# refresh-bio/fqsqueezer

Hardware: AMD Instinct MI355X
Metric: Mbases/s compressed (DNA stream, SE sorted) (higher is better)
Workload: dtype u64; 1 GPU; 1000000x150bp SE, G=7500000 (seed 2+rank), -om s -gs 8 -qm n -im n; workers_T=64, blocks=256, per_gpu=one independent file per GPU

## Files before the change

fqsqueezer_amd/codec.py:

```python
from __future__ import annotations

import ctypes as C
import os
from typing import List, Optional

import numpy as np

_PKG = os.path.dirname(os.path.abspath(__file__))
DEFAULT_LIB = os.path.join(_PKG, "libfqsx.so")

STAT_NAMES = ["gprobe", "gslot", "lprobe", "lslot", "gins", "gins_slot", "siv_words", "ctx_slots",
              "coded", "lins", "mail", "bases", "siv_saved", "dec_refetch"]


class FqsxError(RuntimeError):
    pass


def _load(path: str):
    if not os.path.exists(path):
        raise FqsxError(f"{path} not found: build it with `python -c 'import __graft_entry__ as g; g.build()'` "
                        "(hipcc --offload-arch=gfx950); there is no CPU fallback")
    try:
        import torch
    except ImportError:
        pass
    lib = C.CDLL(path)
    lib.fqsx_dna_create.restype = C.c_int
    lib.fqsx_dna_create.argtypes = [C.c_char_p, C.c_int, C.POINTER(C.c_void_p)]
    if hasattr(lib, "fqsx_dna_create_on_partition"):
        lib.fqsx_dna_create_on_partition.restype = C.c_int
        lib.fqsx_dna_create_on_partition.argtypes = [C.c_char_p, C.c_int, C.c_uint32, C.c_uint32, C.POINTER(C.c_void_p)]
    lib.fqsx_dna_destroy.argtypes = [C.c_void_p]
    lib.fqsx_dna_encode_block.restype = C.c_int
    lib.fqsx_dna_encode_block.argtypes = [C.c_void_p, C.c_void_p, C.c_void_p, C.c_uint32, C.c_uint32,
# ... 759 lines not shown
```

fqsqueezer_amd/csrc/fqsx_dev.h:

```cpp
#pragma once
#include "fqsx_layout.h"
#include "fqsx_rc.h"

#define FQSX_RR 6u
#define FQSX_SW 4u
#define FQSX_NSC 3u
#define FQSX_SCR FQSX_NSC
#define FQSX_RQ 256u
struct SpecBuf {
  u32 h_read, h_i0, h_n;
  u32 h_epoch;
  u32 h_pub;
  u32 h_fix_lane, h_fix_end;
  u32 h_pq_lo[2];
  u32 h_np, h_nlp;
  u64 h_ns, h_nls;
  u64 sp_sdir[6][FQSX_SPEC];
  u64 sp_src[6][FQSX_SPEC];
  u8 sp_scur[6][FQSX_SPEC];
  u64 sp_key[10][FQSX_SPEC];
  u8 sp_kind[FQSX_SPEC];
  u64 sp_cq[FQSX_SPEC];
  u8 sp_lvz[FQSX_SPEC];
  u8 sp_flag[FQSX_SPEC];
  u8 sp_rsym[FQSX_SPEC];
  u8 sp_rep[FQSX_SPEC];
  u8 sp_nrun[FQSX_SPEC];
  u64 pv_b[FQSX_SPEC], pv_s[FQSX_SPEC], pv_pd[FQSX_SPEC], pv_pr[FQSX_SPEC];
  u8 pv_flag[FQSX_SPEC];
  u32 sx_lb[FQSX_SPEC];
  u64 sx_s[FQSX_SPEC];
  u64 sx_ls[FQSX_SPEC];
  u8 sx_flag[FQSX_SPEC];
  u8 rr_idx[FQSX_SPEC];
  u32 rr_front;
  u64 rr_res[FQSX_RR][64];
  u64 rr_hit[FQSX_RR];
  u64 rr_ns[FQSX_RR];
  u64 rc_hit[FQSX_SPEC];
  u64 rc_val[FQSX_SPEC][3];
  u32 rc_ns[FQSX_SPEC];
  u8 ep_off[FQSX_SPEC][2];
  u64 ep_res[64];
  u8 ep_ns[64];
};
#define FQSX_HD_RAW 56u
struct HeadRec {
  u32 idx;
  u32 n_raw, same, n_run, n_p;
  u32 hist[4];
  u64 raw[FQSX_HD_RAW][2];
  u64 pmail[2];
  u64 kdir[3], krc[3];
  u32 kcur[3];
};
struct WgShared {
  HeadRec hd[FQSX_HD];
  u32 hd_ready, hd_taken;
  u32 hd_early;
  alignas(8) u32 mt[4][624];
  u32 mt_idx[4];
  alignas(8) u8 rd[FQSX_HD][FQSX_RD_LDS];
  u64 bk_key[256];
  u32 bk_res[256][4];
  u8 bk_dir[256];
  union {
    SpecBuf sb[1 + FQSX_SCR];
    struct {
// ... 1718 lines not shown
      }
      bool ok = (c[0] | c[1] | c[2] | c[3]) != 0;
      if (m) ok = ok && c[0] <= thr && c[1] <= thr && c[2] <= thr && c[3] <= thr;
      if (!tb) ok = ok && (c[0] == 63) + (c[1] == 63) + (c[2] == 63) + (c[3] == 63) <= 1;
      if (ok) {
        const u32 i = i0 + e;
        const int cor_dist = tb ? (int)cfg->smer : (int)cfg->bmer, d = (int)i - (int)w.cor_pos;
        const u32 cz = d < cor_dist ? (u32)(1 + 2 * (cor_dist - d) / cor_dist) : 0u;
        sb->sp_cq[e] = (u64)c[0] | ((u64)c[1] << 16) | ((u64)c[2] << 32) | ((u64)c[3] << 48);
        sb->sp_lvz[e] = (u8)((tb ? LV_SMER : LV_BMER) | (cz << 4));
        sb->sp_kind[e] = SK_RANK_PENDING;
        sb->sp_rep[e] = 0xff;
        sb->sp_flag[e] = 1;
        const u32 pf = sb->pv_flag[e];
        if (pf & PV_PCAND) sb->pv_flag[e] = (u8)(pf | PV_P);
        np = cnt;
        nsl = nn;
      } else if (!tb && (c[0] | c[1] | c[2] | c[3]) != 0)
        sb->sp_flag[e] = 4;
    }
  }
  np = wave_sum32(np); nsl = wave_sum32(nsl);
  FQ_SYNC();
  if (FQ_LANE == 0) { sb->h_np += np; sb->h_ns += nsl; }
  FQ_SYNC();
}
#endif

FQ_DEV u32 find_counts(Wk &w, C4 &counts, bool b_miss_known, u32 ep = ~0u) {
  const DevCfg *cfg = w.cfg;
  c4_zero(counts);
  u32 bmargin = cfg->bmer - cfg->smer - 1;
  u32 smargin = cfg->smer - cfg->pmer + 1;
  const u32 pre_b = ep != ~0u ? w.sb->ep_off[ep][0] : 0xffu, pre_s = ep != ~0u ? w.sb->ep_off[ep][1] : 0xffu;
  if (km_almost_full(w.bm, cfg->gb, bmargin)) {
    if (!b_miss_known && kt_find(w, cfg->g_b, true, cfg->gb, w.bm, RNG_B, CINC_B, counts, pre_b)) {
      u32 sat = (counts.c[0] == 63) + (counts.c[1] == 63) + (counts.c[2] == 63) + (counts.c[3] == 63);
      if (sat > 1) {
        C4 c2;
        kt_find(w, cfg->g_s, true, cfg->gs, w.sm_, RNG_S, CINC_S, c2);
        counts.c[0] += c2.c[0]; counts.c[1] += c2.c[1]; counts.c[2] += c2.c[2]; counts.c[3] += c2.c[3];
        return LV_MIXED;
      }
      return LV_BMER;
    } else {
      lq_sync_for(w, MAIL_B, cfg->gb, w.bm);
      if (kt_find(w, cfg->l_b, false, cfg->gb, w.bm, RNG_LB, CINC_B, counts)) return LV_BMER;
// ... 208 lines not shown
  return 0xff;
}

struct SpecLane {
  u64 sdir[6], src[6], key[7], pv_b, pv_s, pv_pd, pv_pr, sx_s, sx_ls;
  u32 sx_lb;
  u8 scur[6], nrun, kind, flag, rsym, rep, pv_flag, sx_flag, valid;
};
struct SpecHead { u32 lo0, lo1, np, nlp; u64 ns, nls; };
FQ_DEV void spec_store_lane(SpecBuf *sb, u32 jj, const SpecLane &L) {
  for (u32 x = 0; x < 6; ++x) { sb->sp_sdir[x][jj] = L.sdir[x]; sb->sp_src[x][jj] = L.src[x]; sb->sp_scur[x][jj] = L.scur[x]; }
  sb->sp_nrun[jj] = L.nrun;
  if (L.flag == 1) {
    for (u32 l = 0; l < 7; ++l) sb->sp_key[l][jj] = L.key[l];
    sb->sp_rsym[jj] = L.rsym;
  }
  if (L.flag == 3) { sb->sx_lb[jj] = L.sx_lb; sb->sx_s[jj] = L.sx_s; sb->sx_ls[jj] = L.sx_ls; sb->sx_flag[jj] = L.sx_flag; }
  sb->sp_flag[jj] = L.flag; sb->sp_kind[jj] = L.kind; sb->sp_rep[jj] = L.rep;
  sb->pv_b[jj] = L.pv_b; sb->pv_s[jj] = L.pv_s; sb->pv_pd[jj] = L.pv_pd; sb->pv_pr[jj] = L.pv_pr; sb->pv_flag[jj] = L.pv_flag;
}
FQ_DEV void spec_store_head(SpecBuf *sb, u32 lo0, u32 lo1) {
  if (FQ_LANE == 0) { sb->h_pq_lo[0] = lo0; sb->h_pq_lo[1] = lo1; }
  for (u32 j = FQ_LANE; j < FQSX_SPEC; j += FQ_WAVE) { sb->rr_idx[j] = 0xff; sb->ep_off[j][0] = 0xff; sb->ep_off[j][1] = 0xff; }
  if (FQ_LANE == 0) { sb->rr_front = FQSX_SPEC; sb->h_fix_lane = 0xff; sb->h_fix_end = 0; }
}
FQ_DEV void spec_commit(Wk &w, const SpecLane &L, const SpecHead &H) {
  FQ_SYNC();
  spec_store_head(w.sb, H.lo0, H.lo1);
  if (L.valid) spec_store_lane(w.sb, FQ_LANE, L);
  if (FQ_LANE == 0) { w.sb->h_np = H.np; w.sb->h_nlp = H.nlp; w.sb->h_ns = H.ns; w.sb->h_nls = H.nls; }
  FQ_SYNC();
}
template <bool DEFER>
FQ_DEV bool speculate_t(Wk &w, const u8 *p, u32 size, u32 i0, u32 n, bool reversed, u32 joff, u32 lane0, SpecLane *Lout, SpecHead *Hout) {
  const DevCfg *cfg = w.cfg;
  u64 ns = 0, nls = 0;
  u32 np = 0, nlp = 0;
  const u32 lo0 = lq_done_now(w, 0), lo1 = lq_done_now(w, 1);
  FQ_SYNC();
  if (!DEFER && lane0 == 0) spec_store_head(w.sb, lo0, lo1);
  if (DEFER) Lout->valid = 0;
  const u32 b0 = i0 - joff;
  bool gave_up = false;
  for (u32 j = FQ_LANE; j < n; j += FQ_WAVE) {
    const u32 jj = lane0 + j;
    SpecLane O;
    O.valid = 1; O.sx_lb = 0; O.sx_s = 0; O.sx_ls = 0; O.sx_flag = 0; O.rsym = 0;
// ... 153 lines not shown
    }
    O.pv_b = km_norm(bm, cfg->gb);
    O.pv_s = km_norm(sk, cfg->gs);
    O.pv_pd = km_aligned_dir(pm);
    O.pv_pr = km_aligned_rc(pm);
    O.pv_flag = (u8)pf;
    if (DEFER) *Lout = O; else spec_store_lane(w.sb, jj, O);
  }
  if (wave_any(gave_up)) return false;
  FQ_SYNC();
  np = wave_sum32(np); nlp = wave_sum32(nlp);
  ns = wave_sum64(ns); nls = wave_sum64(nls);
  if (DEFER) { Hout->lo0 = lo0; Hout->lo1 = lo1; Hout->np = np; Hout->nlp = nlp; Hout->ns = ns; Hout->nls = nls; }
  else if (FQ_LANE == 0) {
    if (lane0 == 0) { w.sb->h_np = np; w.sb->h_nlp = nlp; w.sb->h_ns = ns; w.sb->h_nls = nls; }
    else { w.sb->h_np += np; w.sb->h_nlp += nlp; w.sb->h_ns += ns; w.sb->h_nls += nls; }
  }
  FQ_SYNC();
  return true;
}
FQ_DEV bool speculate(Wk &w, const u8 *p, u32 size, u32 i0, u32 n, bool reversed, u32 joff = 0, u32 lane0 = 0) {
  return speculate_t<false>(w, p, size, i0, n, reversed, joff, lane0, nullptr, nullptr);
}
FQ_DEV void spec_adopt(Wk &w) {
  w.pq_lo[0] = w.sb->h_pq_lo[0];
  w.pq_lo[1] = w.sb->h_pq_lo[1];
  w.st[ST_GPROBE] += w.sb->h_np;
  w.st[ST_GSLOT] += w.sb->h_ns;
  w.st[ST_LPROBE] += w.sb->h_nlp;
  w.st[ST_LSLOT] += w.sb->h_nls;
}

FQ_DEV void load_state(Wk &w, u32 j);
FQ_DEV void replace_last_all(Wk &w, u64 symk);
FQ_DEV bool scout_fix(Wk &w, const u8 *p, u32 size, u32 i0, u32 n, bool reversed) {
#if FQ_WAVE > 1
  SpecBuf *sb = w.sb;
  const u32 lane = FQ_LANE;
  FQ_SYNC();
  const bool f = lane < n && sb->sp_flag[lane] == 1, r = f && sb->sp_rep[lane] != 0xff;
  const u64 Fm = wave_ballot(f), Rm = wave_ballot(r);
  if (!Rm) return true;
  const u32 js = ctz64(Rm);
  const u32 lanes_left = FQSX_SPEC - (js + 1), pos_left = size - (i0 + js + 1);
  if ((~Fm & ((1ull << js) - 1ull)) != 0 || lanes_left == 0 || pos_left == 0) return true;
  const Kmer s0 = w.pm, s1 = w.sm_, s2 = w.bm, s3 = w.pm_u, s4 = w.sm_u, s5 = w.bm_u;
  const u32 s_cor = w.cor_pos, s_nrun = w.N_run;
  const u32 sym = rd_sym(w, p, i0 + js, size), rep = sb->sp_rep[js];
  load_state(w, js);
  replace_last_all(w, sym == 4 ? 0 : sym);
  km_replace_last(w.pm, rep); km_replace_last(w.sm_, rep); km_replace_last(w.bm, rep);
  w.cor_pos = i0 + js;
  w.N_run = sym == 4 ? w.N_run + 1 : 0;
// ... 399 lines not shown
      if ((RS >> t) & 1ull) h = 0;
      h = ((h << 1) + ((Z >> t) & 1ull)) & 0xff;
    }
    w.c_r_sym = h;
#endif
  }
#undef CQE
  TM_END_MD(w, TM_SP_HIT, t_rs);
#ifdef FQSX_TIMING_MODELS
  TM_COUNT(w, TM_SP_MISS);
#endif
  TM_END(w, TM_CR_RC, t_rc);
  return L;
}
FQ_DEV u32 cq_process(Wk &w, u32 head, u32 avail) {
  u32 L = code_run(w, head, avail < 64 ? avail : 64);
  if (L == 0) {
    code_one(w, head);
    TM_COUNT(w, CN_P2);
    L = 1;
  }
  return L;
}
FQ_DEV void code_chunk(Wk &w, const u8 *p, u32 size, u32 i0, u32 j0, u32 m, bool reversed, u32 hist_start, bool &first) {
  if (m <= j0) return;
  TM_BEGIN(t_c2);
  WgShared *sm = w.sm;
  code_keys(w, p, size, i0, j0, m, reversed, hist_start);
  TM_END(w, TM_KEYS, t_c2);
  TM_BEGIN(t_cq);
  if (!cq_wait_space(w, m - j0)) return;
  for (u32 j = j0 + FQ_LANE; j < m; j += FQ_WAVE) {
    const u32 e = (w.cq_tail + (j - j0)) & (FQSX_CQ - 1);
    const u32 kind = w.sb->sp_kind[j];
    const u32 nk = kind == SK_LETTER ? 10u : 7u;
    for (u32 l = 0; l < nk; ++l) sm->cq_key[l][e] = w.sb->sp_key[l][j];
    sm->cq_kind[e] = (u8)(kind | (first && j == j0 ? SK_RESET : 0u));
    sm->cq_rsym[e] = w.sb->sp_rsym[j];
  }
  FQ_SYNC();
  first = false;
  cq_publish(w, m - j0);
  TM_END(w, TX_CHUNKQ, t_cq);
  if (!w.piped) {
    while (w.cq_head != w.cq_tail && !w.err) w.cq_head += cq_process(w, w.cq_head, w.cq_tail - w.cq_head);
    TM_END(w, TM_FAST, t_c2);
  }
}

#if FQ_WAVE > 1
FQ_DEV u32 grp_hash(u64 g) { return (u32)((g * 0x9E3779B97F4A7C15ull) >> 52); }
// ... 134 lines not shown
FQ_DEV void scout_restart(Wk &w, u32 read, u32 i0, const u64 s_let[4], u32 flags, bool hold) {
  WgShared *sm = w.sm;
  if (lds_load_acq(&sm->sc_dead)) return;
  const bool in_ring = w.sb != &sm->sb[0];
  const u32 base = in_ring ? ((u32)(w.sb - &sm->sb[1]) + 1u) % w.nsc : 0u;
  hold = hold && in_ring;
  FQ_SYNC();
  if (FQ_LANE == 0) {
    WgShared::ScoutReq &q = sm->sc_req;
    q.slot_base = base;
    q.read = read; q.i0 = i0; q.cor_pos = w.cor_pos; q.n_run = w.N_run;
    q.flags = flags | (w.rq_rev ? (u32)SCQ_REVERSED : 0u); q.size = w.rq_size; q.p = (u64)w.rq_p;
    const Kmer *k[6] = {&w.pm, &w.sm_, &w.bm, &w.pm_u, &w.sm_u, &w.bm_u};
    for (u32 x = 0; x < 6; ++x) { q.kdir[x] = k[x]->dir; q.krc[x] = k[x]->rc; q.kcur[x] = k[x]->cur; }
    for (u32 x = 0; x < 4; ++x) q.s_let[x] = s_let[x];
  }
  w.sc_taken = 0;
  w.sc_base = base;
  FQ_SYNC();
  lds_store_rel(&sm->sc_taken, hold ? 0xffffffffu : 0u);
  w.sc_epoch += 1;
  lds_store_rel(&sm->sc_req_seq, w.sc_epoch);
}
FQ_DEV bool scout_seek(Wk &w, u32 at, const SpecBuf *fixed, u32 fixed_pub) {
  WgShared *sm = w.sm;
  for (;;) {
    SpecBuf *b = &sm->sb[1 + (w.sc_base + w.sc_taken) % w.nsc];
    u32 spins = 0;
    while (lds_load_acq(&b->h_pub) != w.sc_taken + 1 || b->h_epoch != w.sc_epoch) {
      fq_sleep();
      if (lds_load_acq(&sm->sc_dead) || spin_expired(spins)) { w.sc_abandoned = true; return false; }
    }
    const i32 older = (i32)(b->h_read - w.sc_read);
    if (older < 0) { scout_release(w); continue; }
    if (older > 0 || at < b->h_i0) { w.sc_abandoned = true; return false; }
    const u32 lanes = fixed == b && fixed_pub == b->h_pub && b->h_fix_end > b->h_n ? b->h_fix_end : b->h_n;
    if (at < b->h_i0 + lanes) { w.sb = b; return true; }
    scout_release(w);
  }
}

FQ_DEV void suffix(Wk &w, const u8 *p, u32 size, bool original_order, u32 start_pos = 0, bool reversed = false, u32 hist_start = 0) {
  const DevCfg *cfg = w.cfg;
  WgShared *sm = w.sm;
  bool first = true;
  u32 i = start_pos ? start_pos : original_order ? cfg->prefix : cfg->pmer;
  w.rq_p = p; w.rq_size = size; w.rq_rev = reversed;
  if (w.rq_early) w.rq_early = false;
  else if (w.scout && w.sc_reqmode && i < size) {
    w.sc_read += 1;
    w.sc_abandoned = w.rq_noscout;
    if (!w.rq_noscout) scout_restart(w, w.sc_read, i, w.s_let, 0, false);
  }
  w.rq_noscout = false;
  const u32 dbg = cfg->dbg;
  if ((dbg & FQSX_DBG_ABANDON) && w.scout && w.sc_read % 3 == 1) w.sc_abandoned = true;
  u32 at = i;
  u32 own_lo = 0, own_hi = 0;
  const SpecBuf *fixed = nullptr;
  u32 fixed_pub = 0;
  const u32 at_first = at;
  const SpecBuf *counted = nullptr;
  u32 counted_pub = 0;
  while (at < size && !w.err) {
    TM_BEGIN(t_sp);
    if ((dbg & FQSX_DBG_ABANDON) && w.scout && w.sc_read % 3 == 2 && at != at_first) w.sc_abandoned = true;
    bool pre = false;
    u32 n, j0 = 0;
    WHATIF(*w.cfg, 1, 1);
    if (!(at >= own_lo && at < own_hi) && w.scout && !w.sc_abandoned) pre = scout_seek(w, at, fixed, fixed_pub);
    if (pre) {
      const u32 fl = w.sb->h_fix_lane, fe = w.sb->h_fix_end, jx = at - w.sb->h_i0;
      if (fl != 0xff && jx > fl && jx < fe && !(fixed == w.sb && fixed_pub == w.sb->h_pub)) {
        own_lo = at;
        if (own_hi < w.sb->h_i0 + fe) own_hi = w.sb->h_i0 + fe;
        pre = false;
      }
    }
    if (pre) {
      i = w.sb->h_i0; n = w.sb->h_n; j0 = at - i;
      if (fixed == w.sb && fixed_pub == w.sb->h_pub && w.sb->h_fix_end > n) n = w.sb->h_fix_end;
      w.pq_lo[0] = w.sb->h_pq_lo[0];
      w.pq_lo[1] = w.sb->h_pq_lo[1];
      if (counted != w.sb || counted_pub != w.sb->h_pub) { counted = w.sb; counted_pub = w.sb->h_pub; spec_adopt(w); }
    } else {
      i = at;
      n = chunk_len(size - at);
      if (w.scout && !w.sc_abandoned && at >= own_lo && at < own_hi && own_hi - at < n) n = own_hi - at;
      w.sb = &sm->sb[0];
      TM_BEGIN(t_own);
      speculate(w, p, size, i, n, reversed);
      TM_END(w, TX_OWNSPEC, t_own);
      spec_adopt(w);
    }
    TM_END(w, TM_SPEC, t_sp);
    TM_COUNT(w, CN_CHUNK);
    u64 Fm = 0, Rm = 0;
    for (u32 t = FQ_LANE; t < 64; t += FQ_WAVE) {
      const bool f = t < n && w.sb->sp_flag[t] == 1, r = f && w.sb->sp_rep[t] != 0xff;
#if FQ_WAVE > 1
      Fm = wave_ballot(f); Rm = wave_ballot(r);
#else
      Fm |= (u64)f << t; Rm |= (u64)r << t;
#endif
    }
    u64 Qm = 0;
#if FQ_WAVE <= 1
    const u64 NCb = 0, NCs = 0;
#else
    const u64 live = (n >= 64 ? ~0ull : (1ull << n) - 1ull) & (~0ull << j0);
    u64 NCb = 0, NCs = 0;
    if (pre && (live & ~Fm)) {
      TM_BEGIN(t_qm);
      local_refresh(w, j0, n);
      const ConfMasks cmk = conflict_masks(w, n, !w.repm_gate);
      Qm = cmk.quiet; NCb = cmk.ncb; NCs = cmk.ncs;
      TM_END(w, TX_QMM, t_qm);
    }
#endif
#if FQ_WAVE > 1
    u32 pk = 0, pk2 = 4;
    {
      const u32 t = FQ_LANE;
      if (t < n) {
        pk = (u32)w.sb->sp_flag[t] | ((u32)w.sb->sx_flag[t] << 8) | ((u32)w.sb->sp_nrun[t] << 16) | ((u32)w.sb->pv_flag[t] << 24);
        pk2 = (size <= FQSX_RD_LDS && i + t < size ? (u32)w.rdp[i + t] : 4u) | ((u32)w.sb->sp_rep[t] << 8) | ((u32)w.sb->sp_scur[2][t] << 16);
      }
    }
#define PKJ(v, jj) ((u32)__builtin_amdgcn_readlane((int)(v), (int)(jj)))
#endif
    u32 q_done = j0;
    u32 w_pos = j0;
    u32 m = j0;
    bool dirty = false;
    bool foreseen = false;
    for (u32 j = j0; j < n && !dirty && !w.err; ++j) {
      const u32 pos = i + j;
#if FQ_WAVE > 1
      const u32 pkj = PKJ(pk, j), pk2j = PKJ(pk2, j);
      const u32 sym = size <= FQSX_RD_LDS ? (pk2j & 0xffu) : rd_sym(w, p, pos, size);
      const u32 flag = pkj & 0xffu;
#else
      const u32 sym = rd_sym(w, p, pos, size);
      const u32 flag = w.sb->sp_flag[j];
#endif
      const u64 sym_k = sym == 4 ? 0 : sym;
#if FQ_WAVE > 1
      if ((Qm >> j) & 1) {
        TM_BEGIN(t_qr);
        u32 spins = 0, front;
        TM_BEGIN(t_rrw);
        while ((front = lds_load_acq(&w.sb->rr_front)) <= j) {
          fq_sleep();
          if (spin_expired(spins)) { w.err = FQSX_ERR_PIPE; break; }
        }
        TM_END(w, TM_RRWAIT, t_rrw);
        const u32 t = FQ_LANE;
        const u32 form = t < n ? w.sb->rr_idx[t] : 0xffu;
        const bool summed = form == 0xfd;
        const bool empty = t < front && t < n && ((Qm >> t) & 1) && ((form == 0xfe && w.sb->rc_hit[t] == 0) || summed);
        const u64 run = wave_ballot(empty) >> j;
        const u32 len = ~run ? ctz64(~run) : 64u;
        if (len) {
          const bool in = t >= j && t < j + len;
          u32 nsl = 0;
          if (in) {
            if (summed && w.sb->sp_nrun[t] < 2) {
              w.sb->sp_cq[t] = w.sb->rc_val[t][0];
              w.sb->sp_lvz[t] = (u8)(LV_PMER | (3u << 4));
              w.sb->sp_kind[t] = SK_RANK_PENDING;
            } else
              w.sb->sp_kind[t] = SK_LETTER_PENDING;
            const u32 pf = w.sb->pv_flag[t];
            if (pf & PV_PCAND) w.sb->pv_flag[t] = (u8)(pf | PV_P);
            nsl = w.sb->rc_ns[t];
          }
          FQ_SYNC();
          w.st[ST_GPROBE] += (u64)len * 4 * (cfg->gb.k - 1);
          w.st[ST_GSLOT] += wave_sum32(nsl) + (u64)len * (cfg->gb.k - 1);
#ifdef FQSX_TIMING
          w.tm[CN_SLOW] += len; w.tm[CN_EXT] += len; w.tm[CN_ROUGH] += len;
#endif
          j += len - 1;
          m = j + 1;
          TM_END(w, TX_QRUN, t_qr);
          continue;
        }
        TM_END(w, TX_QRUN, t_qr);
      }
#endif
      TM_BEGIN(t_code);
      if (flag == 1) {
        const u64 fm = Fm >> j, rm = Rm >> j;
        const u32 nf = ~fm ? ctz64(~fm) : 64u;
        const u64 rr = nf >= 64 ? rm : rm & ((1ull << nf) - 1ull);
        const u32 len = rr ? ctz64(rr) + 1 : nf;
        j += len - 1;
        const u32 pos = i + j;
#if FQ_WAVE > 1
        const u32 pk2e = PKJ(pk2, j);
        const u32 sym = size <= FQSX_RD_LDS ? (pk2e & 0xffu) : rd_sym(w, p, pos, size);
        const u32 rep = (pk2e >> 8) & 0xffu;
#else
        const u32 sym = rd_sym(w, p, pos, size);
        const u32 rep = w.sb->sp_rep[j];
#endif
        const u64 sym_k = sym == 4 ? 0 : sym;
#ifdef FQSX_TIMING
        w.tm[CN_FAST] += len;
#endif
        if (rep != 0xff) {
          load_state(w, j);
          replace_last_all(w, sym_k);
          flush_pushes(w, q_done, j + 1);
          q_done = j + 1;
          km_replace_last(w.pm, rep); km_replace_last(w.sm_, rep); km_replace_last(w.bm, rep);
          w.cor_pos = pos;
          w.N_run = sym == 4 ? w.N_run + 1 : 0;
          push_b_local(w);
          w_pos = j + 1;
          dirty = true;
          foreseen = true;
        }
      } else {
        C4 counts;
        c4_zero(counts);
#if FQ_WAVE > 1
        u32 level = LV_NONE, nrun_here = (pkj >> 16) & 0xffu;
        const u32 xf = flag == 3 ? (pkj >> 8) & 0xffu : 0u;
        const u32 scur2_j = (pk2j >> 16) & 0xffu;
#else
        u32 level = LV_NONE, nrun_here = w.sb->sp_nrun[j];
        const u32 xf = flag == 3 ? w.sb->sx_flag[j] : 0;
        const u32 scur2_j = w.sb->sp_scur[2][j];
#endif
        bool rough = false, loaded = false, resolved = false;
        TM_COUNT(w, CN_SLOW);
        const bool early_b = flag == 4;
        if (early_b) {
          Kmer bmj;
          bmj.dir = bmj.rc = 0; bmj.cur = scur2_j;
          kt_find(w, cfg->g_b, true, cfg->gb, bmj, RNG_B, CINC_B, counts, w.sb->ep_off[j][0]);
          resolved = true;
// ... 88 lines not shown
          TM_BEGIN(t_fc);
          level = find_counts(w, counts, flag == 3, j);
          TM_END(w, TM_FINDC, t_fc);
          if (level == LV_BMER_UNC) {
            w.bm = w.bm_u; w.sm_ = w.sm_u; w.pm = w.pm_u;
            w.cor_pos = 0;
            level = LV_BMER;
            dirty = true;
          }
          if (level == LV_NONE) {
            TM_BEGIN(t_r);
            TM_COUNT(w, CN_ROUGH);
            if (km_full(w.bm, cfg->gb)) {
              if (rough_kt(w, cfg->g_b, cfg->gb, w.bm, RNG_B, CINC_B, counts)) { level = LV_PMER; rough = true; }
            } else if (km_full(w.sm_, cfg->gs)) {
              if (rough_kt(w, cfg->g_s, cfg->gs, w.sm_, RNG_S, CINC_S, counts)) { level = LV_PMER; rough = true; }
            } else if (km_full(w.pm, cfg->gp)) {
              if (rough_p(w, counts)) { level = LV_PMER; rough = true; }
            }
            TM_END(w, TM_ROUGH, t_r);
          }
        }
        TM_END(w, TM_SPRE, t_code);
        if (level != LV_NONE && nrun_here < 2) {
          int cor_dist = level == LV_PMER ? (int)cfg->pmer : level == LV_SMER ? (int)cfg->smer : (int)cfg->bmer;
          int d = (int)pos - (int)w.cor_pos;
          u32 cor_zone = d < cor_dist ? (u32)(1 + 2 * (cor_dist - d) / cor_dist) : 0u;
          if (rough) cor_zone = 3;
          FQ_SYNC();
          if (FQ_LANE == 0) {
            w.sb->sp_cq[j] = (u64)(counts.c[0] & 0xffff) | ((u64)(counts.c[1] & 0xffff) << 16) | ((u64)(counts.c[2] & 0xffff) << 32) | ((u64)(counts.c[3] & 0xffff) << 48);
            w.sb->sp_lvz[j] = (u8)(level | (cor_zone << 4));
            w.sb->sp_kind[j] = SK_RANK_PENDING;
          }
          FQ_SYNC();
        } else {
          FQ_SYNC();
          if (FQ_LANE == 0) w.sb->sp_kind[j] = SK_LETTER_PENDING;
          FQ_SYNC();
        }
        const bool lvl_sbm = level == LV_SMER || level == LV_BMER || level == LV_MIXED;
        if (loaded) {
          if (sym == 4) ++w.N_run; else w.N_run = 0;
          replace_last_all(w, sym_k);
          u32 pf = 0;
          if (sym < 4) {
// ... 42 lines not shown
            }
            flush_pushes(w, q_done, j + 1);
            q_done = j + 1;
            bool rep;
            if (chk_existing) rep = repair_existing(w, pos, counts, sym);
            else {
              TM_BEGIN(t_rm);
              TM_COUNT(w, CN_REPM);
              rep = repair_missing(w, pos);
              TM_END(w, TM_REPM, t_rm);
            }
            if (rep) {
              push_b_local(w);
              dirty = true;
            }
          }
        }
        TM_END(w, TM_SLOW, t_code);
      }
      m = j + 1;
    }
    if (dirty) TM_COUNT(w, CN_DIRTY);
    { TM_BEGIN(t_fl); flush_pushes(w, q_done, m); TM_END(w, TX_FLUSH, t_fl); }
    code_chunk(w, p, size, i, j0, m, reversed, hist_start, first);
    lq_publish(w);
    if (w_pos != m) {
      const u32 sym = rd_sym(w, p, i + m - 1, size);
      load_state(w, m - 1);
      replace_last_all(w, sym == 4 ? 0 : sym);
      w.N_run = sym == 4 ? w.N_run + 1 : 0;
    }
    at = i + m;
    if (dirty || (dbg & FQSX_DBG_RESTART)) {
      own_lo = at;
      own_hi = at + cfg->bmer - 1;
      if (pre && dirty && foreseen && !(dbg & FQSX_DBG_RESTART) && w.sb->h_fix_lane == m - 1) {
        own_lo = i + w.sb->h_fix_end;
        fixed = w.sb;
        fixed_pub = w.sb->h_pub;
        if (w.sb->h_fix_end > n) n = w.sb->h_fix_end;
      }
    }
    if (pre && m == n) scout_release(w);
  }
}

FQ_DEV bool read_head(Wk &w, const u8 *p, u32 size, const u8 *prev, u32 prev_size, bool first_of_pair, u32 hist[4]) {
  const DevCfg *cfg = w.cfg;
  const bool orig = !first_of_pair || w.mode == 0 || w.mode == 2;
  bool diff = prev == nullptr || prev_size != size;
  u32 h0 = 0, h1 = 0, h2 = 0, h3 = 0;
  FQ_SYNC();
  for (u32 i = FQ_LANE; i < size; i += FQ_WAVE) {
    u8 ch = p[i];
    if (!diff && prev[i] != ch) diff = true;
    u32 c = dna_code(ch);
    if (i < FQSX_RD_LDS) w.rdp[i] = (u8)c;
    h0 += c == 0; h1 += c == 1; h2 += c == 2; h3 += c == 3;
  }
  FQ_SYNC();
  hist[0] = wave_sum32(h0); hist[1] = wave_sum32(h1); hist[2] = wave_sum32(h2); hist[3] = wave_sum32(h3);
  bool same = !wave_any(diff);
  if (prev == nullptr || prev_size != size) same = false;
// ... 458 lines not shown
        spins = 0;
        TM_BEGIN(t_w2);
        while ((i32)(seq - lds_load_acq(&sm->sc_taken)) >= (i32)FQSX_SCR) {
          if (lds_load_acq(&sm->sc_req_seq) != w.sc_epoch) { restart = true; break; }
          fq_sleep();
          if (lds_load_acq(&sm->cq_done) || lds_load_acq(&sm->sc_dead) || spin_expired(spins)) { quit = true; break; }
        }
        TM_END(w, TM_SCOUT_WAIT, t_w2);
        if (quit || restart) break;
        w.sb = &sm->sb[1 + me];
        lds_store_rel(&w.sb->h_pub, 0u);
        spec_commit(w, spl, sph);
        TM_COUNT(w, CN_SC_CHUNK);
#if FQ_WAVE > 1
        TM_BEGIN(t_se);
        if (i0 == base_pos) { scout_early(w, n); scout_settle_early(w, i0, n); }
        TM_END(w, TM_SC_EARLY, t_se);
        if (!scout_fix(w, p, size, i0, n, false)) { TM_COUNT(w, CN_SC_ABORT); restart = true; break; }
        const u32 n_sw = uniform32(w.sb->h_fix_end) > n ? uniform32(w.sb->h_fix_end) : n;
        const u32 front0 = scout_rough_first(w, n_sw);
#else
        const u32 front0 = FQSX_SPEC;
#endif
        if (FQ_LANE == 0) { w.sb->h_read = idx; w.sb->h_i0 = i0; w.sb->h_n = n; w.sb->h_epoch = w.sc_epoch; w.sb->rr_front = front0; }
        FQ_SYNC();
        lds_store_rel(&w.sb->h_pub, seq + 1);
#if FQ_WAVE > 1
        TM_BEGIN(t_sr);
        WHATIF(cfg, 8, 1);
        scout_rough(w, n_sw);
        TM_END(w, TM_SC_ROUGH, t_sr);
#endif
      }
      if (restart || quit) continue;
      add_s_letters(w, hist);
    }
    FQ_SYNC();
    lds_store_rel(&sm->sc_hd_taken[me], idx + 1);
    ++idx;
  }
  if (lds_load_acq(&sm->sc_dead)) lds_store_rel(&sm->sc_hd_taken[me], 0x7fffffffu);
#ifdef FQSX_TIMING
  if (FQ_LANE == 0)
    for (u32 i = 0; i < FQSX_TM_SLOTS && i < 48; ++i) if (w.tm[i]) atomic_add64(&ws->stat[16 + i], w.tm[i]);
#endif
  if (me == 0) TM_STAMP(cfg, tid, launch, 4);
// ... 53 lines not shown
      if (!whole) { TM_COUNT(w, CN_SC_ABORT); break; }
      spins = 0;
      bool stop = false;
      TM_BEGIN(t_w2);
      while ((i32)(seq - lds_load_acq(&sm->sc_taken)) >= (i32)nsc) {
        if (lds_load_acq(&sm->sc_req_seq) != w.sc_epoch || lds_load_acq(&sm->cq_done)) { stop = true; break; }
        fq_sleep();
        if (spin_expired(spins)) { stop = true; break; }
      }
      TM_END(w, TM_SCOUT_WAIT, t_w2);
      if (stop) break;
      w.sb = &sm->sb[1 + me];
      lds_store_rel(&w.sb->h_pub, 0u);
      spec_commit(w, spl, sph);
      TM_COUNT(w, CN_SC_CHUNK);
#if FQ_WAVE > 1
      if (i0 == base_pos) { scout_early(w, n); scout_settle_early(w, i0, n); }
      if (!scout_fix(w, p, size, i0, n, reversed)) { TM_COUNT(w, CN_SC_ABORT); break; }
      const u32 n_sw = uniform32(w.sb->h_fix_end) > n ? uniform32(w.sb->h_fix_end) : n;
      const u32 front0 = scout_rough_first(w, n_sw);
#else
      const u32 front0 = FQSX_SPEC;
#endif
      if (FQ_LANE == 0) { w.sb->h_read = call; w.sb->h_i0 = i0; w.sb->h_n = n; w.sb->h_epoch = w.sc_epoch; w.sb->rr_front = front0; }
      FQ_SYNC();
      lds_store_rel(&w.sb->h_pub, seq + 1);
#if FQ_WAVE > 1
      TM_BEGIN(t_sr);
      scout_rough(w, n_sw);
      TM_END(w, TM_SC_ROUGH, t_sr);
#endif
    }
  }
#ifdef FQSX_TIMING
  if (FQ_LANE == 0)
    for (u32 i = 0; i < FQSX_TM_SLOTS && i < 48; ++i) if (w.tm[i]) atomic_add64(&w.ws->stat[16 + i], w.tm[i]);
#endif
  if (me == 0) TM_STAMP(cfg, tid, launch, 4);
}

template <int MODE, bool DECODE, bool PIPED>
FQ_DEV void encode_segment_body(const DevCfg &cfg, WgShared *sm, u32 tid, u32 n_reads, u32 S, u32 seg, u32 launch = 0) {
  constexpr bool decode = DECODE, piped = PIPED;
  Wk w;
  w.cfg = &cfg;
  w.sm = sm;
// ... 487 lines not shown
```

fqsqueezer_amd/csrc/fqsx_layout.h:

```cpp
#pragma once
#include "fqsx_plat.h"

#define FQSX_MAX_T 255
#define FQSX_SIV_BLK_LOG 14u
#define FQSX_SIV_BLK (1u << FQSX_SIV_BLK_LOG)
#define FQSX_NIL 0xffffffffu
#define FQSX_RD_LDS 3072u
#define FQSX_HD 3u
#define FQSX_SPEC 64u
#define FQSX_PQ 512u
#define FQSX_CQ 256u

struct KGeom {
  u32 k, shift;
  u64 mask, kernel_mask;
};

#define FQSX_BKT 4u
struct KTab {
  u64 *slots;
  u64 nb;
  u64 stride;
  u32 *filled;
  u32 k, cbits;
// ... 58 lines not shown
  u64 rc_low, rc_range;
  u64 out_len;
  u64 dec_buffer, dec_pos;
  u32 mt_idx[4];
  alignas(8) u32 mt[4][624];
  u64 stat[64];
};
enum { RNG_B = 0, RNG_S = 1, RNG_LB = 2, RNG_LS = 3 };
enum {
  ST_GPROBE = 0,
  ST_GSLOT,
  ST_LPROBE,
  ST_LSLOT,
  ST_GINS,
  ST_GINS_SLOT,
  ST_SIV_WORDS,
  ST_CTX,
  ST_CODED,
  ST_LINS,
  ST_MAIL,
  ST_BASES,
  ST_SIV_SAVED,
  ST_DEC_REFETCH,
  ST_N
};
enum { TM_TOTAL = 0, TM_SPEC, TM_FAST, TM_SLOW, TM_POST, TM_READ_HEAD, TM_LQ, TM_ROUGH, TM_REPM, TM_FINDC,
       CN_FAST, CN_SLOW, CN_CHUNK, CN_DIRTY, CN_ROUGH, CN_REPM,
       CN_EXT, CN_GENERIC, CN_LQFLUSH, TM_RRWAIT , TM_CQWAIT , CN_EARLY, CN_P2, TM_P2,
       TM_CODER_IDLE , TM_SCOUT_WAIT , TM_SPRE,
       TM_CR_S, TM_CR_MID, TM_CR_AVG, TM_CR_RC, TM_KEYS,
       TM_SC_SPEC , TM_SC_EARLY, TM_SC_ROUGH , TM_SC_IDLE , CN_SC_CHUNK, CN_SC_ABORT,
       TM_SP_ROLL , TM_SP_PROBE ,
       TM_N, TM_SP_HIT = 46 , TM_SP_MISS = 47 ,
       TX_QMM = 48 , TX_QRUN , TX_PROLOG ,
       TX_CHUNKQ , TX_FLUSH ,
       TX_G_EARLY , TX_OWNSPEC  };
#ifdef FQSX_TIMING
#define FQSX_TM_SLOTS 56
#else
#define FQSX_TM_SLOTS 1
#endif

struct DevCfg {
  u32 T, mode;
  u32 prefix, pmer, smer, bmer;
  KGeom gp, gs, gb;
// ... 31 lines not shown
  u8 *dscratch;
  u64 dcap;
  u8 *pe_scr;
  u64 pe_scr_cap;
  u32 *err;
  u64 *trace;
  u32 shard_rank, shard_world;
  u32 tab_load_pct;
  u32 whatif;
  u32 sys_scope;
  u32 pe_part;
  u32 siv_part, pad_siv_;
  u64 *p_log;
  u32 *p_log_n;
  const u8 *vmap;
  u32 *shard_cnt;
};

enum {
  FQSX_DBG_SCOUTS_OFF = 1,
  FQSX_DBG_ABANDON = 2,
  FQSX_DBG_RESTART = 4,
  FQSX_DBG_INSERTER_STALL = 8,
};
enum {
  FQSX_ERR_OUT_OVERFLOW = 1,
  FQSX_ERR_GTAB_FULL = 2,
  FQSX_ERR_LTAB_FULL = 3,
  FQSX_ERR_CTX_FULL = 4,
  FQSX_ERR_MAIL_FULL = 5,
  FQSX_ERR_PE_FULL = 6,
  FQSX_ERR_PE_READ_TOO_LONG = 7,
  FQSX_ERR_DECODE = 8,
  FQSX_ERR_PIPE = 9,
};
```

Before: 109.8 Mbases/s.

## Snapshot scout chunk header into registers and continue in place at fix lane

Scout chunk headers now sit in one dword block and are read in a single LDS load per lane, then broadcast with readlane into a register copy. The flag and repeat masks are computed once by the producer (spec_digest) rather than by the coder on every chunk. When the scout's fix lane is reached, the coder now flushes the coded prefix and keeps going in the same chunk instead of marking it dirty and restarting. A kpend flag lets code_keys be skipped when no key work is pending. This removes repeated LDS header reads and chunk restarts, at the cost of more complex control flow and a double-checked publish handshake.

```diff
diff --git a/fqsqueezer_amd/codec.py b/fqsqueezer_amd/codec.py
--- a/fqsqueezer_amd/codec.py
+++ b/fqsqueezer_amd/codec.py
@@ -10,7 +10,7 @@
 DEFAULT_LIB = os.path.join(_PKG, "libfqsx.so")
 
 STAT_NAMES = ["gprobe", "gslot", "lprobe", "lslot", "gins", "gins_slot", "siv_words", "ctx_slots",
-              "coded", "lins", "mail", "bases", "siv_saved", "dec_refetch"]
+              "coded", "lins", "mail", "bases", "siv_saved", "dec_refetch", "inplace"]
 
 
 class FqsxError(RuntimeError):
diff --git a/fqsqueezer_amd/csrc/fqsx_dev.h b/fqsqueezer_amd/csrc/fqsx_dev.h
--- a/fqsqueezer_amd/csrc/fqsx_dev.h
+++ b/fqsqueezer_amd/csrc/fqsx_dev.h
@@ -7,14 +7,22 @@
 #define FQSX_NSC 3u
 #define FQSX_SCR FQSX_NSC
 #define FQSX_RQ 256u
+#define FQSX_HDR_DW 20u
 struct SpecBuf {
-  u32 h_read, h_i0, h_n;
-  u32 h_epoch;
-  u32 h_pub;
-  u32 h_fix_lane, h_fix_end;
-  u32 h_pq_lo[2];
-  u32 h_np, h_nlp;
-  u64 h_ns, h_nls;
+  union {
+    struct {
+      u32 h_read, h_i0, h_n;
+      u32 h_epoch;
+      u32 h_pub;
+      u32 h_fix_lane, h_fix_end;
+      u32 h_pq_lo[2];
+      u32 h_np, h_nlp;
+      u32 h_kpend;
+      u64 h_ns, h_nls;
+      u64 h_Fm, h_Rm;
+    };
+    u32 h_w[FQSX_HDR_DW];
+  };
   u64 sp_sdir[6][FQSX_SPEC];
   u64 sp_src[6][FQSX_SPEC];
   u8 sp_scur[6][FQSX_SPEC];
@@ -44,6 +52,7 @@
   u64 ep_res[64];
   u8 ep_ns[64];
 };
+static_assert(__builtin_offsetof(SpecBuf, sp_sdir) == 4u * FQSX_HDR_DW && __builtin_offsetof(SpecBuf, h_Rm) == 4u * (FQSX_HDR_DW - 2u), "SpecBuf: the header is one block of FQSX_HDR_DW dwords");
 #define FQSX_HD_RAW 56u
 struct HeadRec {
   u32 idx;
@@ -1808,7 +1817,7 @@
   }
   np = wave_sum32(np); nsl = wave_sum32(nsl);
   FQ_SYNC();
-  if (FQ_LANE == 0) { sb->h_np += np; sb->h_ns += nsl; }
+  if (FQ_LANE == 0) { sb->h_np += np; sb->h_ns += nsl; if (np) sb->h_kpend = 1; }
   FQ_SYNC();
 }
 #endif
@@ -2063,7 +2072,20 @@
 FQ_DEV void spec_store_head(SpecBuf *sb, u32 lo0, u32 lo1) {
   if (FQ_LANE == 0) { sb->h_pq_lo[0] = lo0; sb->h_pq_lo[1] = lo1; }
   for (u32 j = FQ_LANE; j < FQSX_SPEC; j += FQ_WAVE) { sb->rr_idx[j] = 0xff; sb->ep_off[j][0] = 0xff; sb->ep_off[j][1] = 0xff; }
-  if (FQ_LANE == 0) { sb->rr_front = FQSX_SPEC; sb->h_fix_lane = 0xff; sb->h_fix_end = 0; }
+  if (FQ_LANE == 0) { sb->rr_front = FQSX_SPEC; sb->h_fix_lane = 0xff; sb->h_fix_end = 0; sb->h_kpend = 0; }
+}
+FQ_DEV void spec_digest(SpecBuf *sb) {
+  FQ_SYNC();
+  u64 Fm = 0, Rm = 0;
+  for (u32 t = FQ_LANE; t < 64; t += FQ_WAVE) {
+    const bool f = sb->sp_flag[t] == 1, r = f && sb->sp_rep[t] != 0xff;
+#if FQ_WAVE > 1
+    Fm = wave_ballot(f); Rm = wave_ballot(r);
+#else
+    Fm |= (u64)f << t; Rm |= (u64)r << t;
+#endif
+  }
+  if (FQ_LANE == 0) { sb->h_Fm = Fm; sb->h_Rm = Rm; }
 }
 FQ_DEV void spec_commit(Wk &w, const SpecLane &L, const SpecHead &H) {
   FQ_SYNC();
@@ -2263,13 +2285,41 @@
 FQ_DEV bool speculate(Wk &w, const u8 *p, u32 size, u32 i0, u32 n, bool reversed, u32 joff = 0, u32 lane0 = 0) {
   return speculate_t<false>(w, p, size, i0, n, reversed, joff, lane0, nullptr, nullptr);
 }
-FQ_DEV void spec_adopt(Wk &w) {
-  w.pq_lo[0] = w.sb->h_pq_lo[0];
-  w.pq_lo[1] = w.sb->h_pq_lo[1];
-  w.st[ST_GPROBE] += w.sb->h_np;
-  w.st[ST_GSLOT] += w.sb->h_ns;
-  w.st[ST_LPROBE] += w.sb->h_nlp;
-  w.st[ST_LSLOT] += w.sb->h_nls;
+struct ChunkHdr {
+  u32 read, i0, n, epoch, pub, fix_lane, fix_end, lo0, lo1, np, nlp, kpend;
+  u64 ns, nls, Fm, Rm;
+};
+struct ChunkTake {
+  ChunkHdr h;
+  u32 pk, pk2;
+};
+FQ_DEV void chunk_take(const SpecBuf *b, ChunkTake &T) {
+#if FQ_WAVE > 1
+  const u32 t = FQ_LANE;
+  const u32 hv = b->h_w[t < FQSX_HDR_DW ? t : 0u];
+  T.pk = (u32)b->sp_flag[t] | ((u32)b->sx_flag[t] << 8) | ((u32)b->sp_nrun[t] << 16) | ((u32)b->pv_flag[t] << 24);
+  T.pk2 = ((u32)b->sp_rep[t] << 8) | ((u32)b->sp_scur[2][t] << 16);
+#define HDW(k) ((u32)__builtin_amdgcn_readlane((int)hv, (int)(k)))
+#define HDQ(k) ((u64)HDW(k) | ((u64)HDW((k) + 1) << 32))
+  ChunkHdr &h = T.h;
+  h.read = HDW(0); h.i0 = HDW(1); h.n = HDW(2); h.epoch = HDW(3); h.pub = HDW(4); h.fix_lane = HDW(5); h.fix_end = HDW(6);
+  h.lo0 = HDW(7); h.lo1 = HDW(8); h.np = HDW(9); h.nlp = HDW(10); h.kpend = HDW(11);
+  h.ns = HDQ(12); h.nls = HDQ(14); h.Fm = HDQ(16); h.Rm = HDQ(18);
+#undef HDQ
+#undef HDW
+#else
+  ChunkHdr &h = T.h;
+  h.read = b->h_read; h.i0 = b->h_i0; h.n = b->h_n; h.epoch = b->h_epoch; h.pub = b->h_pub; h.fix_lane = b->h_fix_lane; h.fix_end = b->h_fix_end;
+  h.lo0 = b->h_pq_lo[0]; h.lo1 = b->h_pq_lo[1]; h.np = b->h_np; h.nlp = b->h_nlp; h.kpend = b->h_kpend;
+  h.ns = b->h_ns; h.nls = b->h_nls; h.Fm = b->h_Fm; h.Rm = b->h_Rm;
+  T.pk = T.pk2 = 0;
+#endif
+}
+FQ_DEV void spec_adopt(Wk &w, const ChunkHdr &h) {
+  w.st[ST_GPROBE] += h.np;
+  w.st[ST_GSLOT] += h.ns;
+  w.st[ST_LPROBE] += h.nlp;
+  w.st[ST_LSLOT] += h.nls;
 }
 
 FQ_DEV void load_state(Wk &w, u32 j);
@@ -2715,11 +2765,11 @@
   }
   return L;
 }
-FQ_DEV void code_chunk(Wk &w, const u8 *p, u32 size, u32 i0, u32 j0, u32 m, bool reversed, u32 hist_start, bool &first) {
+FQ_DEV void code_chunk(Wk &w, const u8 *p, u32 size, u32 i0, u32 j0, u32 m, bool reversed, u32 hist_start, bool &first, bool keys) {
   if (m <= j0) return;
   TM_BEGIN(t_c2);
   WgShared *sm = w.sm;
-  code_keys(w, p, size, i0, j0, m, reversed, hist_start);
+  if (keys) code_keys(w, p, size, i0, j0, m, reversed, hist_start);
   TM_END(w, TM_KEYS, t_c2);
   TM_BEGIN(t_cq);
   if (!cq_wait_space(w, m - j0)) return;
@@ -2900,20 +2950,31 @@
   w.sc_epoch += 1;
   lds_store_rel(&sm->sc_req_seq, w.sc_epoch);
 }
-FQ_DEV bool scout_seek(Wk &w, u32 at, const SpecBuf *fixed, u32 fixed_pub) {
+FQ_DEV bool scout_seek(Wk &w, u32 at, const SpecBuf *fixed, u32 fixed_pub, ChunkTake &T) {
   WgShared *sm = w.sm;
   for (;;) {
     SpecBuf *b = &sm->sb[1 + (w.sc_base + w.sc_taken) % w.nsc];
     u32 spins = 0;
-    while (lds_load_acq(&b->h_pub) != w.sc_taken + 1 || b->h_epoch != w.sc_epoch) {
+    for (;;) {
+      if (lds_load_acq(&b->h_pub) == w.sc_taken + 1) {
+        chunk_take(b, T);
+        if (T.h.epoch == w.sc_epoch) {
+          if (w.sc_taken >= w.nsc) break;
+          if (lds_load_acq(&b->h_pub) == w.sc_taken + 1) {
+            chunk_take(b, T);
+            if (T.h.epoch == w.sc_epoch) break;
+          }
+        }
+      }
       fq_sleep();
       if (lds_load_acq(&sm->sc_dead) || spin_expired(spins)) { w.sc_abandoned = true; return false; }
     }
-    const i32 older = (i32)(b->h_read - w.sc_read);
+    const ChunkHdr &h = T.h;
+    const i32 older = (i32)(h.read - w.sc_read);
     if (older < 0) { scout_release(w); continue; }
-    if (older > 0 || at < b->h_i0) { w.sc_abandoned = true; return false; }
-    const u32 lanes = fixed == b && fixed_pub == b->h_pub && b->h_fix_end > b->h_n ? b->h_fix_end : b->h_n;
-    if (at < b->h_i0 + lanes) { w.sb = b; return true; }
+    if (older > 0 || at < h.i0) { w.sc_abandoned = true; return false; }
+    const u32 lanes = fixed == b && fixed_pub == h.pub && h.fix_end > h.n ? h.fix_end : h.n;
+    if (at < h.i0 + lanes) { w.sb = b; return true; }
     scout_release(w);
   }
 }
@@ -2931,7 +2992,7 @@
     if (!w.rq_noscout) scout_restart(w, w.sc_read, i, w.s_let, 0, false);
   }
   w.rq_noscout = false;
-  const u32 dbg = cfg->dbg;
+  const u32 dbg = cfg->dbg | FQSX_DBG_ALWAYS;
   if ((dbg & FQSX_DBG_ABANDON) && w.scout && w.sc_read % 3 == 1) w.sc_abandoned = true;
   u32 at = i;
   u32 own_lo = 0, own_hi = 0;
@@ -2946,21 +3007,24 @@
     bool pre = false;
     u32 n, j0 = 0;
     WHATIF(*w.cfg, 1, 1);
-    if (!(at >= own_lo && at < own_hi) && w.scout && !w.sc_abandoned) pre = scout_seek(w, at, fixed, fixed_pub);
+    ChunkTake T;
+#if FQ_WAVE > 1
+    const u32 sv = size <= FQSX_RD_LDS && at + FQ_LANE < size ? (u32)w.rdp[at + FQ_LANE] : 4u;
+#define PKJ(v, jj) ((u32)__builtin_amdgcn_readlane((int)(v), (int)(jj)))
+#endif
+    if (!(at >= own_lo && at < own_hi) && w.scout && !w.sc_abandoned) pre = scout_seek(w, at, fixed, fixed_pub, T);
     if (pre) {
-      const u32 fl = w.sb->h_fix_lane, fe = w.sb->h_fix_end, jx = at - w.sb->h_i0;
-      if (fl != 0xff && jx > fl && jx < fe && !(fixed == w.sb && fixed_pub == w.sb->h_pub)) {
+      const u32 fl = T.h.fix_lane, fe = T.h.fix_end, jx = at - T.h.i0;
+      if (fl != 0xff && jx > fl && jx < fe && !(fixed == w.sb && fixed_pub == T.h.pub)) {
         own_lo = at;
-        if (own_hi < w.sb->h_i0 + fe) own_hi = w.sb->h_i0 + fe;
+        if (own_hi < T.h.i0 + fe) own_hi = T.h.i0 + fe;
         pre = false;
       }
     }
     if (pre) {
-      i = w.sb->h_i0; n = w.sb->h_n; j0 = at - i;
-      if (fixed == w.sb && fixed_pub == w.sb->h_pub && w.sb->h_fix_end > n) n = w.sb->h_fix_end;
-      w.pq_lo[0] = w.sb->h_pq_lo[0];
-      w.pq_lo[1] = w.sb->h_pq_lo[1];
-      if (counted != w.sb || counted_pub != w.sb->h_pub) { counted = w.sb; counted_pub = w.sb->h_pub; spec_adopt(w); }
+      i = T.h.i0; n = T.h.n; j0 = at - i;
+      if (fixed == w.sb && fixed_pub == T.h.pub && T.h.fix_end > n) n = T.h.fix_end;
+      if (counted != w.sb || counted_pub != T.h.pub) { counted = w.sb; counted_pub = T.h.pub; spec_adopt(w, T.h); }
     } else {
       i = at;
       n = chunk_len(size - at);
@@ -2969,44 +3033,37 @@
       TM_BEGIN(t_own);
       speculate(w, p, size, i, n, reversed);
       TM_END(w, TX_OWNSPEC, t_own);
-      spec_adopt(w);
-    }
+      spec_digest(w.sb);
+      FQ_SYNC();
+      chunk_take(w.sb, T);
+      spec_adopt(w, T.h);
+    }
+    const ChunkHdr &H = T.h;
+    w.pq_lo[0] = H.lo0;
+    w.pq_lo[1] = H.lo1;
     TM_END(w, TM_SPEC, t_sp);
     TM_COUNT(w, CN_CHUNK);
-    u64 Fm = 0, Rm = 0;
-    for (u32 t = FQ_LANE; t < 64; t += FQ_WAVE) {
-      const bool f = t < n && w.sb->sp_flag[t] == 1, r = f && w.sb->sp_rep[t] != 0xff;
-#if FQ_WAVE > 1
-      Fm = wave_ballot(f); Rm = wave_ballot(r);
-#else
-      Fm |= (u64)f << t; Rm |= (u64)r << t;
-#endif
-    }
+    u64 lanes_n = n >= 64 ? ~0ull : (1ull << n) - 1ull;
+    u64 Fm = H.Fm & lanes_n, Rm = H.Rm & lanes_n;
     u64 Qm = 0;
 #if FQ_WAVE <= 1
     const u64 NCb = 0, NCs = 0;
 #else
-    const u64 live = (n >= 64 ? ~0ull : (1ull << n) - 1ull) & (~0ull << j0);
     u64 NCb = 0, NCs = 0;
-    if (pre && (live & ~Fm)) {
+    if (pre && (lanes_n & (~0ull << j0) & ~Fm)) {
       TM_BEGIN(t_qm);
       local_refresh(w, j0, n);
       const ConfMasks cmk = conflict_masks(w, n, !w.repm_gate);
       Qm = cmk.quiet; NCb = cmk.ncb; NCs = cmk.ncs;
       TM_END(w, TX_QMM, t_qm);
     }
-#endif
-#if FQ_WAVE > 1
-    u32 pk = 0, pk2 = 4;
-    {
-      const u32 t = FQ_LANE;
-      if (t < n) {
-        pk = (u32)w.sb->sp_flag[t] | ((u32)w.sb->sx_flag[t] << 8) | ((u32)w.sb->sp_nrun[t] << 16) | ((u32)w.sb->pv_flag[t] << 24);
-        pk2 = (size <= FQSX_RD_LDS && i + t < size ? (u32)w.rdp[i + t] : 4u) | ((u32)w.sb->sp_rep[t] << 8) | ((u32)w.sb->sp_scur[2][t] << 16);
-      }
-    }
-#define PKJ(v, jj) ((u32)__builtin_amdgcn_readlane((int)(v), (int)(jj)))
-#endif
+    u32 pk = T.pk;
+    const u32 pk2 = T.pk2;
+    if (pre && (lanes_n & (~0ull << j0) & ~Fm)) pk = (pk & ~0xff00u) | ((u32)w.sb->sx_flag[FQ_LANE] << 8);
+#endif
+    const u32 jb = j0;
+    u32 jc = j0;
+    bool kp = H.kpend != 0;
     u32 q_done = j0;
     u32 w_pos = j0;
     u32 m = j0;
@@ -3016,7 +3073,7 @@
       const u32 pos = i + j;
 #if FQ_WAVE > 1
       const u32 pkj = PKJ(pk, j), pk2j = PKJ(pk2, j);
-      const u32 sym = size <= FQSX_RD_LDS ? (pk2j & 0xffu) : rd_sym(w, p, pos, size);
+      const u32 sym = size <= FQSX_RD_LDS ? PKJ(sv, j - jb) : rd_sym(w, p, pos, size);
       const u32 flag = pkj & 0xffu;
 #else
       const u32 sym = rd_sym(w, p, pos, size);
@@ -3059,6 +3116,7 @@
 #ifdef FQSX_TIMING
           w.tm[CN_SLOW] += len; w.tm[CN_EXT] += len; w.tm[CN_ROUGH] += len;
 #endif
+          kp = true;
           j += len - 1;
           m = j + 1;
           TM_END(w, TX_QRUN, t_qr);
@@ -3077,7 +3135,7 @@
         const u32 pos = i + j;
 #if FQ_WAVE > 1
         const u32 pk2e = PKJ(pk2, j);
-        const u32 sym = size <= FQSX_RD_LDS ? (pk2e & 0xffu) : rd_sym(w, p, pos, size);
+        const u32 sym = size <= FQSX_RD_LDS ? PKJ(sv, j - jb) : rd_sym(w, p, pos, size);
         const u32 rep = (pk2e >> 8) & 0xffu;
 #else
         const u32 sym = rd_sym(w, p, pos, size);
@@ -3097,6 +3155,36 @@
           w.N_run = sym == 4 ? w.N_run + 1 : 0;
           push_b_local(w);
           w_pos = j + 1;
+          if (pre && H.fix_lane == j && !(dbg & (FQSX_DBG_RESTART | FQSX_DBG_NO_INPLACE | FQSX_DBG_ABANDON))) {
+            m = j + 1;
+            code_chunk(w, p, size, i, jc, m, reversed, hist_start, first, kp);
+            jc = m;
+            kp = H.kpend != 0;
+            lq_publish(w);
+            own_lo = i + H.fix_end;
+            own_hi = i + m + cfg->bmer - 1;
+            fixed = w.sb;
+            fixed_pub = H.pub;
+            if (H.fix_end > n) n = H.fix_end;
+            lanes_n = n >= 64 ? ~0ull : (1ull << n) - 1ull;
+            Fm = H.Fm & lanes_n; Rm = H.Rm & lanes_n;
+            w.pq_lo[0] = H.lo0;
+            w.pq_lo[1] = H.lo1;
+            Qm = 0;
+#if FQ_WAVE > 1
+            NCb = NCs = 0;
+            if (lanes_n & (~0ull << m) & ~Fm) {
+              TM_BEGIN(t_qm);
+              local_refresh(w, m, n);
+              const ConfMasks cmk = conflict_masks(w, n, !w.repm_gate);
+              Qm = cmk.quiet; NCb = cmk.ncb; NCs = cmk.ncs;
+              TM_END(w, TX_QMM, t_qm);
+              pk = (pk & ~0xff00u) | ((u32)w.sb->sx_flag[FQ_LANE] << 8);
+            }
+#endif
+            w.st[ST_INPLACE] += 1;
+            continue;
+          }
           dirty = true;
           foreseen = true;
         }
@@ -3231,6 +3319,7 @@
           }
         }
         TM_END(w, TM_SPRE, t_code);
+        kp = true;
         if (level != LV_NONE && nrun_here < 2) {
           int cor_dist = level == LV_PMER ? (int)cfg->pmer : level == LV_SMER ? (int)cfg->smer : (int)cfg->bmer;
           int d = (int)pos - (int)w.cor_pos;
@@ -3319,7 +3408,7 @@
     }
     if (dirty) TM_COUNT(w, CN_DIRTY);
     { TM_BEGIN(t_fl); flush_pushes(w, q_done, m); TM_END(w, TX_FLUSH, t_fl); }
-    code_chunk(w, p, size, i, j0, m, reversed, hist_start, first);
+    code_chunk(w, p, size, i, jc, m, reversed, hist_start, first, kp);
     lq_publish(w);
     if (w_pos != m) {
       const u32 sym = rd_sym(w, p, i + m - 1, size);
@@ -3331,11 +3420,11 @@
     if (dirty || (dbg & FQSX_DBG_RESTART)) {
       own_lo = at;
       own_hi = at + cfg->bmer - 1;
-      if (pre && dirty && foreseen && !(dbg & FQSX_DBG_RESTART) && w.sb->h_fix_lane == m - 1) {
-        own_lo = i + w.sb->h_fix_end;
+      if (pre && dirty && foreseen && !(dbg & FQSX_DBG_RESTART) && H.fix_lane == m - 1) {
+        own_lo = i + H.fix_end;
         fixed = w.sb;
-        fixed_pub = w.sb->h_pub;
-        if (w.sb->h_fix_end > n) n = w.sb->h_fix_end;
+        fixed_pub = H.pub;
+        if (H.fix_end > n) n = H.fix_end;
       }
     }
     if (pre && m == n) scout_release(w);
@@ -3840,6 +3929,7 @@
 #else
         const u32 front0 = FQSX_SPEC;
 #endif
+        spec_digest(w.sb);
         if (FQ_LANE == 0) { w.sb->h_read = idx; w.sb->h_i0 = i0; w.sb->h_n = n; w.sb->h_epoch = w.sc_epoch; w.sb->rr_front = front0; }
         FQ_SYNC();
         lds_store_rel(&w.sb->h_pub, seq + 1);
@@ -3939,6 +4029,7 @@
 #else
       const u32 front0 = FQSX_SPEC;
 #endif
+      spec_digest(w.sb);
       if (FQ_LANE == 0) { w.sb->h_read = call; w.sb->h_i0 = i0; w.sb->h_n = n; w.sb->h_epoch = w.sc_epoch; w.sb->rr_front = front0; }
       FQ_SYNC();
       lds_store_rel(&w.sb->h_pub, seq + 1);
diff --git a/fqsqueezer_amd/csrc/fqsx_layout.h b/fqsqueezer_amd/csrc/fqsx_layout.h
--- a/fqsqueezer_amd/csrc/fqsx_layout.h
+++ b/fqsqueezer_amd/csrc/fqsx_layout.h
@@ -104,6 +104,7 @@
   ST_BASES,
   ST_SIV_SAVED,
   ST_DEC_REFETCH,
+  ST_INPLACE,
   ST_N
 };
 enum { TM_TOTAL = 0, TM_SPEC, TM_FAST, TM_SLOW, TM_POST, TM_READ_HEAD, TM_LQ, TM_ROUGH, TM_REPM, TM_FINDC,
@@ -181,7 +182,11 @@
   FQSX_DBG_ABANDON = 2,
   FQSX_DBG_RESTART = 4,
   FQSX_DBG_INSERTER_STALL = 8,
-};
+  FQSX_DBG_NO_INPLACE = 16,
+};
+#ifndef FQSX_DBG_ALWAYS
+#define FQSX_DBG_ALWAYS 0u
+#endif
 enum {
   FQSX_ERR_OUT_OVERFLOW = 1,
   FQSX_ERR_GTAB_FULL = 2,
```

After: 110.1 Mbases/s, median of 2. About the same (+0.3%).
